# zqs01/ASR_chinese_e2e

Hardware: AMD Instinct MI355X
Metric: training throughput (utterances/s; frames/s = x T), AISHELL-1-shaped 80-mel T=500 (higher is better)
Workload: dtype bf16; 1 GPU; configs[2]: joint CTC/attention (lambda=0.3) encoder-decoder, bf16, per-GPU batch 32, T=500, F=80, V=4232, 6 layers, d_model 512, 8x64 heads, ff 1024, dropout 0.0, fwd+loss+CER+bwd+clip+Noam/Adam per step, eager launches; global_batch=32, seq_len=500, parallelism=dp1

## Files before the change

### asr_chinese_e2e_amd/csrc/asr_common.h

```cpp
#pragma once
#include <hip/hip_runtime.h>
#include <stdint.h>
#include <stdio.h>
#include <string.h>

#include <hip/hip_ext.h>

#include "../../include/asr_hip.h"

typedef __bf16 bf16_t;
typedef __attribute__((ext_vector_type(2))) float f32x2;
typedef __attribute__((ext_vector_type(4))) float f32x4;
typedef __attribute__((ext_vector_type(16))) float f32x16;
typedef __attribute__((ext_vector_type(4))) __bf16 bf16x4;
typedef __attribute__((ext_vector_type(8))) __bf16 bf16x8;
typedef __attribute__((ext_vector_type(4))) unsigned int u32x4;
typedef __attribute__((ext_vector_type(2))) unsigned int u32x2;

#define WAVE 64

void asr_set_error(const char* fmt, ...);
int asr_deterministic(void);
enum { ASR_OPT_CU_LIMIT = 0, ASR_OPT_TN_MULTI = 1, ASR_OPT_SDPA_PAIR = 2, ASR_OPT_SDPA_SMALL = 3, ASR_OPT_COUNT = 4 };
int asr_option(int key);
int asr_option_set(int key, int value);
#define ASR_FAIL(code, ...)        \
    do {                           \
        asr_set_error(__VA_ARGS__); \
        return (code);             \
    } while (0)
#define ASR_CHECK_LAUNCH(name)                                                        \
    do {                                                                              \
        hipError_t e__ = hipGetLastError();                                           \
        if (e__ != hipSuccess) ASR_FAIL(ASR_EHIP, "%s: %s", name, hipGetErrorString(e__)); \
    } while (0)

template <typename T> __device__ __forceinline__ float to_f32(T v);
template <> __device__ __forceinline__ float to_f32<float>(float v) { return v; }
template <> __device__ __forceinline__ float to_f32<bf16_t>(bf16_t v) { return (float)v; }
template <typename T> __device__ __forceinline__ T from_f32(float v);
template <> __device__ __forceinline__ float from_f32<float>(float v) { return v; }
template <> __device__ __forceinline__ bf16_t from_f32<bf16_t>(float v) { return (bf16_t)v; }

template <typename T> __device__ __forceinline__ f32x4 load4(const T* p);
template <> __device__ __forceinline__ f32x4 load4<float>(const float* p) { return *(const f32x4*)p; }
template <> __device__ __forceinline__ f32x4 load4<bf16_t>(const bf16_t* p) {
    bf16x4 v = *(const bf16x4*)p;
    f32x4 r = {(float)v[0], (float)v[1], (float)v[2], (float)v[3]};
    return r;
}
template <typename V> __device__ __forceinline__ void stream_store(V v, V* p) { __builtin_nontemporal_store(v, p); }
template <typename T> __device__ __forceinline__ void store4(T* p, f32x4 v);
template <> __device__ __forceinline__ void store4<float>(float* p, f32x4 v) { *(f32x4*)p = v; }
template <> __device__ __forceinline__ void store4<bf16_t>(bf16_t* p, f32x4 v) {
    bf16x4 r = {(bf16_t)v[0], (bf16_t)v[1], (bf16_t)v[2], (bf16_t)v[3]};
    *(bf16x4*)p = r;
}
template <typename T> __device__ __forceinline__ void load8(const T* p, float (&r)[8]);
template <> __device__ __forceinline__ void load8<float>(const float* p, float (&r)[8]) {
    f32x4 a = *(const f32x4*)p, b = *(const f32x4*)(p + 4);
#pragma unroll
    for (int i = 0; i < 4; ++i) { r[i] = a[i]; r[4 + i] = b[i]; }
}
template <> __device__ __forceinline__ void load8<bf16_t>(const bf16_t* p, float (&r)[8]) {
    bf16x8 v = *(const bf16x8*)p;
#pragma unroll
    for (int i = 0; i < 8; ++i) r[i] = (float)v[i];
}
template <typename T> __device__ __forceinline__ void store8(T* p, const float (&r)[8]);
template <> __device__ __forceinline__ void store8<float>(float* p, const float (&r)[8]) {
    f32x4 a = {r[0], r[1], r[2], r[3]}, b = {r[4], r[5], r[6], r[7]};
    *(f32x4*)p = a;
    *(f32x4*)(p + 4) = b;
}
template <> __device__ __forceinline__ void store8<bf16_t>(bf16_t* p, const float (&r)[8]) {
    bf16x8 v;
#pragma unroll
    for (int i = 0; i < 8; ++i) v[i] = (bf16_t)r[i];
    *(bf16x8*)p = v;
}

#define ASR_FULL_WAVES(threads) static_assert((threads) % 64 == 0, "wave_sum / wave_max need full 64-lane waves: block sizes must be multiples of 64")
template <int CTRL, int ROW_MASK = 0xf>
__device__ __forceinline__ float wave_dpp(float v) {
    return __int_as_float(__builtin_amdgcn_update_dpp(0, __float_as_int(v), CTRL, ROW_MASK, 0xf, true));
}
__device__ __forceinline__ float wave_sum(float v) {
    v += wave_dpp<0xB1>(v);
    v += wave_dpp<0x4E>(v);
    v += wave_dpp<0x141>(v);
    v += wave_dpp<0x140>(v);
    v += wave_dpp<0x142, 0xA>(v);
    v += wave_dpp<0x143, 0xC>(v);
    return __int_as_float(__builtin_amdgcn_readlane(__float_as_int(v), 63));
}
__device__ __forceinline__ float wave_max(float v) {
    v = fmaxf(v, __int_as_float(__builtin_amdgcn_update_dpp(__float_as_int(v), __float_as_int(v), 0xB1, 0xf, 0xf, false)));
    v = fmaxf(v, __int_as_float(__builtin_amdgcn_update_dpp(__float_as_int(v), __float_as_int(v), 0x4E, 0xf, 0xf, false)));
    v = fmaxf(v, __int_as_float(__builtin_amdgcn_update_dpp(__float_as_int(v), __float_as_int(v), 0x141, 0xf, 0xf, false)));
    v = fmaxf(v, __int_as_float(__builtin_amdgcn_update_dpp(__float_as_int(v), __float_as_int(v), 0x140, 0xf, 0xf, false)));
    v = fmaxf(v, __int_as_float(__builtin_amdgcn_update_dpp(__float_as_int(v), __float_as_int(v), 0x142, 0xA, 0xf, false)));
    v = fmaxf(v, __int_as_float(__builtin_amdgcn_update_dpp(__float_as_int(v), __float_as_int(v), 0x143, 0xC, 0xf, false)));
    return __int_as_float(__builtin_amdgcn_readlane(__float_as_int(v), 63));
}
__device__ __forceinline__ float block_sum(float v, float* red) {
    v = wave_sum(v);
// ... 91 lines not shown
```

### asr_chinese_e2e_amd/csrc/gemm.hip

```cpp
#include <stdlib.h>

#include <type_traits>

#include "asr_common.h"

namespace {

static int unsafe_debug_env(const char* name) {
#ifdef ASR_DEBUG_SWITCHES
    const char* e = getenv(name);
    return e ? atoi(e) : 0;
#else
    (void)name;
    return 0;
#endif
}

typedef __attribute__((address_space(3))) bf16x4 lds_bf16x4;
constexpr int BM = 128, BN = 128, BK = 64;
constexpr int AS = 72;

__device__ __forceinline__ int acc_row(int reg, int lane) { return (reg & 3) + 8 * (reg >> 2) + 4 * (lane >> 5); }

struct Stage4 { u32x4 v[4]; };
// ... 323 lines not shown
                            const uint32_t hi_ = ((h & 0x7fff0000u) != 0u && !(h & 0x80000000u)) ? 0xffff0000u : 0u;
                            v[q][e] &= lo_ | hi_;
                        }
                }
#pragma unroll
                for (int q = 0; q < 4; ++q) {
                    const int row = q * 8 + srow, ch = lane & 7;
                    const int m = m0 + mi * 32 + row, n = n0 + ch * 8;
                    bf16_t* rowp = C + (size_t)(m0 + mi * 32 + q * 8) * ldc + n0;
                    if constexpr (decltype(full_c)::value) stream_store(v[q], (u32x4*)((char*)rowp + lane_off));
                    else if (m < M && n + 8 <= N) stream_store(v[q], (u32x4*)((char*)rowp + lane_off));
                }
                __builtin_amdgcn_wave_barrier();
            }
        };
        if (full) store_tail(std::true_type{});
        else store_tail(std::false_type{});
    }
}

template <int ACT, bool KRAG = false>
static void launch_nt_spec(const bf16_t* a, const bf16_t* w, const float* bias, bf16_t* c, int M, int N, int K, int lda, int ldb, int ldc, hipStream_t st,
                           const bf16_t* mask = nullptr, const void* zero_page = nullptr) {
    static bool attr = false;
    if (!attr) {
        (void)hipFuncSetAttribute((const void*)gemm_nt_spec_kernel<ACT, KRAG>, hipFuncAttributeMaxDynamicSharedMemorySize, PLDS);
        attr = true;
    }
    const int t_n = ceil_div(N, PBN), t_m = ceil_div(M, PBM), ntiles = t_n * t_m;
    const int grid = ntiles < cu_count() ? ntiles : cu_count();
    asr_launch_armed(gemm_nt_spec_kernel<ACT, KRAG>, dim3(grid), dim3(512), PLDS, st, a, w, bias, c, M, N, K, lda, ldb, ldc, t_n, ntiles, mask, zero_page);
}

constexpr int SM = 64, SS = 72;
constexpr int SK = 256;
constexpr int SAS = SK + 8;
constexpr int S_A = SM * SAS;
constexpr int S_BT = SK * SS;
struct StageK { u32x4 v[8]; };
__device__ __forceinline__ void sk_load_rows(StageK& st, const bf16_t* __restrict__ base, size_t ld, int row0, int rows, int c0, int cols, int tid) {
#pragma unroll
    for (int c = 0; c < 8; ++c) {
        const int id = tid + 256 * c, row = id >> 5, ch = id & 31;
        const int gr = row0 + row, gc = c0 + ch * 8;
        const u32x4 z = {0u, 0u, 0u, 0u};
        st.v[c] = (gr < rows && gc < cols) ? *(const u32x4*)(base + (size_t)gr * ld + gc) : z;
    }
}
__device__ __forceinline__ void sk_store_rows(const StageK& st, bf16_t* tile, int tid) {
#pragma unroll
    for (int c = 0; c < 8; ++c) {
        const int id = tid + 256 * c, row = id >> 5, ch = id & 31;
        *(u32x4*)(tile + row * SAS + ch * 8) = st.v[c];
    }
}
__device__ __forceinline__ void sk_load_cols(StageK& st, const bf16_t* __restrict__ base, size_t ld, int row0, int rows, int c0, int cols, int tid) {
#pragma unroll
    for (int c = 0; c < 8; ++c) {
        const int id = tid + 256 * c, row = id >> 3, ch = id & 7;
        const int gr = row0 + row, gc = c0 + ch * 8;
        const u32x4 z = {0u, 0u, 0u, 0u};
        st.v[c] = (gr < rows && gc < cols) ? *(const u32x4*)(base + (size_t)gr * ld + gc) : z;
    }
}
__device__ __forceinline__ void sk_store_cols(const StageK& st, bf16_t* tile, int tid) {
#pragma unroll
    for (int c = 0; c < 8; ++c) {
        const int id = tid + 256 * c, row = id >> 3, ch = id & 7;
        *(u32x4*)(tile + row * SS + ch * 8) = st.v[c];
    }
}
__device__ __forceinline__ bf16x8 sm_frag_tr(const bf16_t* tile, int col0, int s, int lane) {
    const int G = lane >> 4, i = lane & 15;
    const bf16_t* p = tile + (16 * s + 8 * (G >> 1) + (i >> 2)) * SS + col0 + 16 * (G & 1) + 4 * (i & 3);
    const bf16x4 lo = __builtin_amdgcn_ds_read_tr16_b64_v4bf16((lds_bf16x4*)p);
    const bf16x4 hi = __builtin_amdgcn_ds_read_tr16_b64_v4bf16((lds_bf16x4*)(p + 4 * SS));
    return __builtin_shufflevector(lo, hi, 0, 1, 2, 3, 4, 5, 6, 7);
}

template <bool TB>
constexpr int small_lds_bytes() { return 2 * (S_A + (TB ? S_BT : S_A)) * 2; }

template <bool TB, int ACT>
__global__ __launch_bounds__(256) void gemm_small_kernel(const bf16_t* __restrict__ A, const bf16_t* __restrict__ Bm, const float* __restrict__ bias,
                                                         const bf16_t* __restrict__ mask, bf16_t* __restrict__ C, int M, int N, int K, int lda, int ldb,
                                                         int ldc, int tiles_n) {
    extern __shared__ __attribute__((aligned(16))) char smem_s[];
    constexpr int BUF = S_A + (TB ? S_BT : S_A);
    bf16_t* smem = (bf16_t*)smem_s;
    const int tid = threadIdx.x, lane = tid & 63, w = tid >> 6;
    const int tn = blockIdx.x % tiles_n, tm = blockIdx.x / tiles_n;
    const int m0 = tm * SM, n0 = tn * SM;
    const int wm = w >> 1, wn = w & 1, r = lane & 31, hh = lane >> 5;
    f32x16 acc[2];
#pragma unroll
    for (int i = 0; i < 16; ++i) { acc[0][i] = 0.f; acc[1][i] = 0.f; }
    StageK sa0, sb0, sa1, sb1;
#define SK_LOAD(SA_, SB_, K0_)                                                                 \
    {                                                                                          \
        sk_load_rows(SA_, A, lda, m0, M, (K0_), K, tid);                                       \
        if (TB) sk_load_cols(SB_, Bm, ldb, (K0_), K, n0, N, tid);    \
        else sk_load_rows(SB_, Bm, ldb, n0, N, (K0_), K, tid);       \
    }
#define SK_STORE(SA_, SB_, BUF_)                                                               \
    {                                                                                          \
        sk_store_rows(SA_, (BUF_), tid);                                                       \
        if (TB) sk_store_cols(SB_, (BUF_) + S_A, tid);                                         \
        else sk_store_rows(SB_, (BUF_) + S_A, tid);                                            \
    }
#define SK_MMA(KT_)                                                                                                                   \
    {                                                                                                                                 \
        const bf16_t* As = smem + ((KT_) & 1) * BUF;                                                                                  \
        const bf16_t* Bs = As + S_A;                                                                                                  \
             \
             \
        _Pragma("unroll") for (int ks = 0; ks < SK / 16; ++ks) {                                                                      \
            const bf16x8 af = *(const bf16x8*)(As + (wm * 32 + r) * SAS + 16 * ks + 8 * hh);                                          \
            const bf16x8 bf = TB ? sm_frag_tr(Bs, wn * 32, ks, lane) : *(const bf16x8*)(Bs + (wn * 32 + r) * SAS + 16 * ks + 8 * hh); \
            acc[ks & 1] = __builtin_amdgcn_mfma_f32_32x32x16_bf16(bf, af, acc[ks & 1], 0, 0, 0);                                      \
        }                                                                                                                             \
    }
    const int nk = (K + SK - 1) / SK;
    SK_LOAD(sa0, sb0, 0);
    if (nk > 1) SK_LOAD(sa1, sb1, SK);
    SK_STORE(sa0, sb0, smem);
    __syncthreads();
    for (int kt = 0; kt < nk; kt += 2) {
        if (kt + 2 < nk) SK_LOAD(sa0, sb0, (kt + 2) * SK);
        SK_MMA(kt);
        if (kt + 1 < nk) SK_STORE(sa1, sb1, smem + BUF);
        __syncthreads();
        if (kt + 1 >= nk) break;
        if (kt + 3 < nk) SK_LOAD(sa1, sb1, (kt + 3) * SK);
        SK_MMA(kt + 1);
        if (kt + 2 < nk) SK_STORE(sa0, sb0, smem);
        __syncthreads();
    }
#undef SK_LOAD
#undef SK_STORE
#undef SK_MMA
    const int m = m0 + wm * 32 + r;
    if (m >= M) return;
#pragma unroll
    for (int g4 = 0; g4 < 4; ++g4) {
        const int n = n0 + wn * 32 + 8 * g4 + 4 * hh;
        if (n >= N) continue;
        f32x4 o;
#pragma unroll
        for (int e = 0; e < 4; ++e) {
            float x = acc[0][4 * g4 + e] + acc[1][4 * g4 + e] + (bias ? bias[n + e] : 0.f);
            if (ACT == ASR_ACT_RELU) x = fmaxf(x, 0.f);
            o[e] = x;
        }
        if (ACT == ASR_ACT_RELU_MASK) {
            const f32x4 h4 = load4<bf16_t>(mask + (size_t)m * ldc + n);
#pragma unroll
            for (int e = 0; e < 4; ++e) o[e] = h4[e] > 0.f ? o[e] : 0.f;
        }
        store4<bf16_t>(C + (size_t)m * ldc + n, o);
    }
}

constexpr int TM = 64;

constexpr int TSTAGE = 2 * TM * 256;
__device__ __attribute__((aligned(256))) unsigned tn_zero_page[64];

template <int OFF>
__device__ __forceinline__ bf16x4 lds_tr16(unsigned addr) {
    bf16x4 v;
    asm volatile("ds_read_b64_tr_b16 %0, %1 offset:%2" : "=v"(v) : "v"(addr), "n"(OFF) : "memory");
    return v;
}
__device__ __forceinline__ unsigned tn_frag_off(int col0, int lane) {
    const int G = lane >> 4, i = lane & 15;
    const int row = 4 * (G >> 1) + (i >> 2);
    const int chunk = ((col0 >> 3) + 2 * (G & 1) + ((i & 3) >> 1)) ^ (4 * ((i >> 2) & 3));
    return (unsigned)(row * 256 + (chunk << 4) + 8 * (i & 1));
}
template <int S>
__device__ __forceinline__ bf16x8 tn_frag_swz(unsigned addr) {
    const bf16x4 lo = lds_tr16<S * 4096>(addr), hi = lds_tr16<S * 4096 + 2048>(addr);
    return __builtin_shufflevector(lo, hi, 0, 1, 2, 3, 4, 5, 6, 7);
}

template <int TRING>
__device__ __forceinline__ void tn_dma_tile(char* smem_t, const bf16_t* __restrict__ dY, const bf16_t* __restrict__ X, float* __restrict__ dW, int N, int K, int ldy,
                                            int ldx, int ldw, int n0, int k0, int tk, int mbeg, int mend, int use_atomic, const void* __restrict__ zero_page,
                                            float* __restrict__ dbias, int split, int bias_split_stride) {
    const int tid = threadIdx.x, lane = tid & 63, w = __builtin_amdgcn_readfirstlane(tid >> 6);
    constexpr int SR = TM;
    constexpr int SBYTES = TSTAGE;
    const int nsteps = (mend - mbeg + SR - 1) / SR;
    if (nsteps <= 0) return;
    const int wn = w >> 1, wk = w & 1;

    const int lrow = lane >> 4, slot = lane & 15;
    const bool is_y = w < 2;
    const bf16_t* cur[8];
    int prow[8];
#pragma unroll
    for (int j = 0; j < 8; ++j) {
        const int gg = (w & 1) * 8 + j;
        const int row = 4 * gg + lrow;
        const int col = (slot ^ (4 * (row & 3))) * 8;
        prow[j] = row;
        cur[j] = is_y ? dY + (size_t)(mbeg + row) * ldy + min(n0 + col, N - 8) : X + (size_t)(mbeg + row) * ldx + min(k0 + col, K - 8);
    }
    const size_t stage_step = (size_t)SR * (is_y ? ldy : ldx);
    const bool ragged = ((mend - mbeg) % SR) != 0;
    int it = 0, it_slot = 0;
    auto fix_last = [&]() {
        if (ragged && it == nsteps - 1) {
#pragma unroll
            for (int j = 0; j < 8; ++j) cur[j] = (mbeg + it * SR + prow[j] < mend) ? cur[j] : (const bf16_t*)zero_page;
        }
    };
    fix_last();
    auto dma = [&](int j) {
        __builtin_amdgcn_global_load_lds((gbl_void_t*)cur[j], (lds_void_t*)(smem_t + it_slot * SBYTES + (w * 8 + j) * 1024), 16, 0, 0);
    };
    auto advance = [&]() {
        ++it;
        it_slot = it_slot == TRING - 1 ? 0 : it_slot + 1;
#pragma unroll
        for (int j = 0; j < 8; ++j) cur[j] += stage_step;
        fix_last();
    };

    f32x16 acc[2][2];
#pragma unroll
    for (int a = 0; a < 2; ++a)
#pragma unroll
        for (int b = 0; b < 2; ++b)
#pragma unroll
            for (int e = 0; e < 16; ++e) acc[a][b][e] = 0.f;
    const unsigned lds_base = (unsigned)(size_t)(__attribute__((address_space(3))) char*)smem_t;
    const unsigned y_off[2] = {tn_frag_off(wn * 64, lane), tn_frag_off(wn * 64 + 32, lane)};
// ... 410 lines not shown
#pragma unroll
            for (int e = 0; e < 4; ++e) t[e] += v[e];
        }
        const size_t n = (i * 4) / K, k = i * 4 - n * K;
        float* dst = dW + n * ldw + k;
#pragma unroll
        for (int e = 0; e < 4; ++e) dst[e] = accumulate ? dst[e] + t[e] : t[e];
    }
}

static int tn_splits(int M, int N, int K) {
    const int tiles = ceil_div(N, 128) * ceil_div(K, 128);
    int s = ceil_div(256, tiles);
    const int max_s = ceil_div(M, 4 * TM);
    if (s > max_s) s = max_s;
    if (s < 1) s = 1;
    return s;
}

}

extern "C" int asr_gemm_nt_bf16(const void* A, const void* W, const float* bias, const void* res, void* C, int M, int N, int K, int lda, int ldb, int ldc,
                                int act, void* stream) {
    if (!A || !W || !C) ASR_FAIL(ASR_EINVAL, "asr_gemm_nt_bf16: null pointer");
    if (M <= 0 || N <= 0 || K <= 0) ASR_FAIL(ASR_EINVAL, "asr_gemm_nt_bf16: bad shape M=%d N=%d K=%d", M, N, K);
    if (K % 8 || lda % 8 || ldb % 8 || ldc % 4 || lda < K || ldb < K || ldc < N) ASR_FAIL(ASR_EINVAL, "asr_gemm_nt_bf16: K, lda, ldb must be multiples of 8 and ldc of 4 (K=%d lda=%d ldb=%d ldc=%d)", K, lda, ldb, ldc);
    if ((((uintptr_t)A | (uintptr_t)W) % 16) || ((uintptr_t)C % 8) || (res && (uintptr_t)res % 8) || (bias && (uintptr_t)bias % 16)) ASR_FAIL(ASR_EINVAL, "asr_gemm_nt_bf16: misaligned pointer");
    hipStream_t st = (hipStream_t)stream;
    if (act != ASR_ACT_RELU && act != ASR_ACT_NONE && act != ASR_ACT_RELU_MASK) ASR_FAIL(ASR_EINVAL, "asr_gemm_nt_bf16: unknown activation %d", act);
    const bool rows16 = N % 8 == 0 && ldc % 8 == 0 && ((uintptr_t)C % 16) == 0;
    if (act == ASR_ACT_RELU_MASK) {
        if (!res || (uintptr_t)res % 16 || K % DBK || K < 2 * PBK || !rows16)
            ASR_FAIL(ASR_EINVAL, "asr_gemm_nt_bf16: ASR_ACT_RELU_MASK needs the mask in `res`, K %% 64 == 0, K >= 128, N, ldc %% 8 == 0 and 16-byte aligned pointers");
        if (bias) ASR_FAIL(ASR_EINVAL, "asr_gemm_nt_bf16: ASR_ACT_RELU_MASK takes no bias");
        launch_nt_spec<ASR_ACT_RELU_MASK>((const bf16_t*)A, (const bf16_t*)W, nullptr, (bf16_t*)C, M, N, K, lda, ldb, ldc, st, (const bf16_t*)res);
        ASR_CHECK_LAUNCH("asr_gemm_nt_bf16");
        return ASR_OK;
    }
    if (res && act == ASR_ACT_NONE && !bias && K % DBK == 0 && K >= 2 * PBK && rows16 && ((uintptr_t)res % 16) == 0) {
        launch_nt_spec<NT_ACT_ADD_RES>((const bf16_t*)A, (const bf16_t*)W, nullptr, (bf16_t*)C, M, N, K, lda, ldb, ldc, st, (const bf16_t*)res);
        ASR_CHECK_LAUNCH("asr_gemm_nt_bf16");
        return ASR_OK;
    }
    if (K % DBK != 0 && K > PBK && !res && act == ASR_ACT_NONE && rows16) {
        static void* zero_page = nullptr;
        if (!zero_page && (hipGetSymbolAddress(&zero_page, HIP_SYMBOL(tn_zero_page)) != hipSuccess || !zero_page))
            ASR_FAIL(ASR_EINVAL, "asr_gemm_nt_bf16: zero page symbol not found");
        launch_nt_spec<ASR_ACT_NONE, true>((const bf16_t*)A, (const bf16_t*)W, bias, (bf16_t*)C, M, N, K, lda, ldb, ldc, st, nullptr, zero_page);
        ASR_CHECK_LAUNCH("asr_gemm_nt_bf16");
        return ASR_OK;
    }
    if (K % DBK == 0 && K >= 2 * PBK && !res && rows16) {
        if (act == ASR_ACT_RELU) launch_nt_spec<ASR_ACT_RELU>((const bf16_t*)A, (const bf16_t*)W, bias, (bf16_t*)C, M, N, K, lda, ldb, ldc, st);
        else launch_nt_spec<ASR_ACT_NONE>((const bf16_t*)A, (const bf16_t*)W, bias, (bf16_t*)C, M, N, K, lda, ldb, ldc, st);
        ASR_CHECK_LAUNCH("asr_gemm_nt_bf16");
        return ASR_OK;
    }
    const int tiles_n = ceil_div(N, BN), tiles_m = ceil_div(M, BM);
    if (act == ASR_ACT_RELU)
        gemm_nt_kernel<ASR_ACT_RELU><<<tiles_n * tiles_m, 256, 0, st>>>((const bf16_t*)A, (const bf16_t*)W, bias, (const bf16_t*)res, (bf16_t*)C, M, N, K, lda, ldb, ldc, tiles_n);
    else if (act == ASR_ACT_NONE)
        gemm_nt_kernel<ASR_ACT_NONE><<<tiles_n * tiles_m, 256, 0, st>>>((const bf16_t*)A, (const bf16_t*)W, bias, (const bf16_t*)res, (bf16_t*)C, M, N, K, lda, ldb, ldc, tiles_n);
    else
        ASR_FAIL(ASR_EINVAL, "asr_gemm_nt_bf16: unknown activation %d", act);
    ASR_CHECK_LAUNCH("asr_gemm_nt_bf16");
    return ASR_OK;
}

extern "C" int asr_gemm_small_bf16(const void* A, const void* Bm, const float* bias, const void* mask, void* C, int M, int N, int K, int lda, int ldb, int ldc,
                                   int trans_b, int act, void* stream) {
    if (!A || !Bm || !C) ASR_FAIL(ASR_EINVAL, "asr_gemm_small_bf16: null pointer");
    if (M <= 0 || N <= 0 || K <= 0) ASR_FAIL(ASR_EINVAL, "asr_gemm_small_bf16: bad shape M=%d N=%d K=%d", M, N, K);
    if (N % 8 || K % 8 || lda % 8 || ldb % 8 || ldc % 4 || lda < K || ldc < N || ldb < (trans_b ? N : K))
        ASR_FAIL(ASR_EINVAL, "asr_gemm_small_bf16: N, K, lda, ldb must be multiples of 8, ldc of 4 (N=%d K=%d lda=%d ldb=%d ldc=%d)", N, K, lda, ldb, ldc);
    if ((((uintptr_t)A | (uintptr_t)Bm) % 16) || ((uintptr_t)C % 8) || (mask && (uintptr_t)mask % 8) || (bias && (uintptr_t)bias % 4)) ASR_FAIL(ASR_EINVAL, "asr_gemm_small_bf16: misaligned pointer");
    if (act != ASR_ACT_NONE && act != ASR_ACT_RELU && act != ASR_ACT_RELU_MASK) ASR_FAIL(ASR_EINVAL, "asr_gemm_small_bf16: unknown activation %d", act);
    if ((act == ASR_ACT_RELU_MASK) != (mask != nullptr)) ASR_FAIL(ASR_EINVAL, "asr_gemm_small_bf16: ASR_ACT_RELU_MASK needs the activations in `mask` (and only it)");
    hipStream_t st = (hipStream_t)stream;
    const int tiles_n = ceil_div(N, SM), grid = tiles_n * ceil_div(M, SM);
    const bf16_t *a = (const bf16_t*)A, *b = (const bf16_t*)Bm, *mk = (const bf16_t*)mask;
    bf16_t* c = (bf16_t*)C;
    static bool attr = false;
    if (!attr) {
        (void)hipFuncSetAttribute((const void*)gemm_small_kernel<true, ASR_ACT_RELU_MASK>, hipFuncAttributeMaxDynamicSharedMemorySize, small_lds_bytes<true>());
        (void)hipFuncSetAttribute((const void*)gemm_small_kernel<true, ASR_ACT_RELU>, hipFuncAttributeMaxDynamicSharedMemorySize, small_lds_bytes<true>());
        (void)hipFuncSetAttribute((const void*)gemm_small_kernel<true, ASR_ACT_NONE>, hipFuncAttributeMaxDynamicSharedMemorySize, small_lds_bytes<true>());
        (void)hipFuncSetAttribute((const void*)gemm_small_kernel<false, ASR_ACT_RELU_MASK>, hipFuncAttributeMaxDynamicSharedMemorySize, small_lds_bytes<false>());
        (void)hipFuncSetAttribute((const void*)gemm_small_kernel<false, ASR_ACT_RELU>, hipFuncAttributeMaxDynamicSharedMemorySize, small_lds_bytes<false>());
        (void)hipFuncSetAttribute((const void*)gemm_small_kernel<false, ASR_ACT_NONE>, hipFuncAttributeMaxDynamicSharedMemorySize, small_lds_bytes<false>());
        attr = true;
    }
#define SMALL(TB_, ACT_) asr_launch_armed(gemm_small_kernel<TB_, ACT_>, dim3(grid), dim3(256), small_lds_bytes<TB_>(), st, a, b, bias, mk, c, M, N, K, lda, ldb, ldc, tiles_n)
    if (trans_b) {
        if (act == ASR_ACT_RELU_MASK) SMALL(true, ASR_ACT_RELU_MASK);
        else if (act == ASR_ACT_RELU) SMALL(true, ASR_ACT_RELU);
        else SMALL(true, ASR_ACT_NONE);
    } else {
        if (act == ASR_ACT_RELU_MASK) SMALL(false, ASR_ACT_RELU_MASK);
        else if (act == ASR_ACT_RELU) SMALL(false, ASR_ACT_RELU);
        else SMALL(false, ASR_ACT_NONE);
    }
#undef SMALL
    ASR_CHECK_LAUNCH("asr_gemm_small_bf16");
    return ASR_OK;
}

namespace {
static void tn_stagger(int M, int rows_per_split, int nsplit, int* r0, int* skew) {
    *r0 = rows_per_split;
    *skew = 0;
    if (nsplit >= 3) {
        int sk = (int)((long long)rows_per_split * 50 / 100 / (nsplit - 1)) / TM * TM;
        const int tri = nsplit * (nsplit - 1) / 2;
        int r = ceil_div(ceil_div(M - sk * tri > 0 ? M - sk * tri : M, nsplit), TM) * TM;
        if (sk <= 0 || r < 4 * TM || r * (nsplit - 1) + sk * ((nsplit - 1) * (nsplit - 2) / 2) >= M) return;
        *r0 = r;
        *skew = sk;
    }
}

static bool tn_multi_launch(const asr_tn_problem* probs, int nprob, int accumulate, hipStream_t st, void* zero_page) {
    if (!asr_option(ASR_OPT_TN_MULTI) || nprob > TNM_MAX || probs[0].M < 4096) return false;
    TnMulti g;
    memset(&g, 0, sizeof(g));
    int tiles = 0;
    for (int i = 0; i < nprob; ++i) {
        const asr_tn_problem& q = probs[i];
        if (q.M != probs[0].M) return false;
        TnMultiProb& t = g.p[i];
        t.dY = (const bf16_t*)q.dY; t.X = (const bf16_t*)q.X; t.dW = q.dW; t.dbias = q.dbias;
        t.N = q.N; t.K = q.K; t.ldy = q.ldy; t.ldx = q.ldx; t.ldw = q.ldw;
        t.tiles_k = ceil_div(q.K, 128);
        t.tiles = ceil_div(q.N, 128) * t.tiles_k;
        tiles += t.tiles;
    }
    const int cus = cu_count(), M = probs[0].M;
    int splits = cus / tiles;
    const int max_s = ceil_div(M, 4 * TM);
    if (splits > max_s) splits = max_s;
    if (splits < 1) splits = 1;
    if (tiles * splits * 5 < cus * 4 && splits < max_s) return false;
    const int rows_per_split = ceil_div(ceil_div(M, splits), TM) * TM;
    g.nsplit = ceil_div(M, rows_per_split);
    g.nprob = nprob;
    g.M = M;
    tn_stagger(M, rows_per_split, g.nsplit, &g.r0, &g.skew);
    int begin = 0;
    for (int i = 0; i < nprob; ++i) {
        g.p[i].block_begin = begin;
        begin += g.p[i].tiles * g.nsplit;
        if (!accumulate) {
            const size_t total = (size_t)g.p[i].N * g.p[i].K;
            const int zg = (int)((total + 255) / 256);
            zero_f32_kernel<<<zg < 1024 ? zg : 1024, 256, 0, st>>>(g.p[i].dW, g.p[i].N, g.p[i].K, g.p[i].ldw);
        }
    }
    static bool attr = false;
    if (!attr) { (void)hipFuncSetAttribute((const void*)gemm_tn_multi_kernel<3>, hipFuncAttributeMaxDynamicSharedMemorySize, 3 * TSTAGE); attr = true; }
    gemm_tn_multi_kernel<3><<<begin, 256, 3 * TSTAGE, st>>>(g, zero_page);
    return true;
}
}

extern "C" int asr_gemm_tn_grouped_bf16(const asr_tn_problem* probs, int nprob, int accumulate, void* stream) {
    if (!probs || nprob <= 0 || nprob > TG_MAX) ASR_FAIL(ASR_EINVAL, "asr_gemm_tn_grouped_bf16: 1..%d problems per call (got %d)", TG_MAX, nprob);
    if (asr_deterministic()) ASR_FAIL(ASR_EINVAL, "asr_gemm_tn_grouped_bf16: the grouped kernel combines splits with fp32 atomics - in deterministic mode call asr_gemm_tn_bias_bf16 per problem");
    hipStream_t st = (hipStream_t)stream;
    TnGroup g;
    memset(&g, 0, sizeof(g));
    g.nprob = nprob;
    long long work = 0;
    int max_m = 0;
    for (int i = 0; i < nprob; ++i) {
        const asr_tn_problem& q = probs[i];
        if (!q.dY || !q.X || !q.dW) ASR_FAIL(ASR_EINVAL, "asr_gemm_tn_grouped_bf16: null pointer in problem %d", i);
// ... 143 lines not shown
```

### asr_chinese_e2e_amd/csrc/misc.hip

```cpp
#include <stdarg.h>
#include <stdlib.h>

#include "asr_common.h"

static thread_local char g_err[512] = "";

void asr_set_error(const char* fmt, ...) {
    va_list ap;
    va_start(ap, fmt);
    vsnprintf(g_err, sizeof(g_err), fmt, ap);
    va_end(ap);
}

extern "C" int asr_abi_version(void) { return ASR_ABI_VERSION; }

static int g_deterministic = -1;
int asr_deterministic(void) {
    if (g_deterministic < 0) {
        const char* e = getenv("ASR_DETERMINISTIC");
        g_deterministic = (e && atoi(e) != 0) ? 1 : 0;
    }
    return g_deterministic;
}
extern "C" int asr_get_deterministic(void) { return asr_deterministic(); }
extern "C" int asr_set_deterministic(int on) {
    const int old = asr_deterministic();
    g_deterministic = on ? 1 : 0;
    return old;
}

static const char* const g_opt_names[ASR_OPT_COUNT] = {"cu_limit", "tn_multi", "sdpa_pair", "sdpa_small"};
static int g_opt_val[ASR_OPT_COUNT] = {0, 1, 0, 1};
static void opt_init() {}
int asr_option(int key) {
    opt_init();
    return (key >= 0 && key < ASR_OPT_COUNT) ? g_opt_val[key] : 0;
}
int asr_option_set(int key, int value) {
    opt_init();
    if (key < 0 || key >= ASR_OPT_COUNT) return 0;
    const int old = g_opt_val[key];
    g_opt_val[key] = value;
    return old;
}
extern "C" int asr_set_option(const char* name, int value, int* previous) {
    opt_init();
    if (!name) ASR_FAIL(ASR_EINVAL, "asr_set_option: null name");
    for (int i = 0; i < ASR_OPT_COUNT; ++i)
        if (strcmp(name, g_opt_names[i]) == 0) {
            if (previous) *previous = g_opt_val[i];
            g_opt_val[i] = value;
            return ASR_OK;
        }
    ASR_FAIL(ASR_EINVAL, "asr_set_option: unknown option '%s'", name);
}

extern "C" int asr_last_error(char* buf, size_t n) {
    if (buf && n) {
        strncpy(buf, g_err, n - 1);
        buf[n - 1] = 0;
    }
    return (int)strlen(g_err);
}

static unsigned fork_event_flags() { return hipEventDisableTiming | hipEventReleaseToDevice; }
static hipEvent_t g_fork_events[256];
static unsigned g_fork_next = 0;
static bool g_fork_init = false;
extern "C" int asr_stream_fork(void* from_stream, void* to_stream) {
    if (!g_fork_init) {
        for (int i = 0; i < 256; ++i)
            if (hipEventCreateWithFlags(&g_fork_events[i], fork_event_flags()) != hipSuccess) ASR_FAIL(ASR_EHIP, "asr_stream_fork: hipEventCreateWithFlags failed");
        g_fork_init = true;
    }
    hipEvent_t ev = g_fork_events[g_fork_next++ & 255u];
    hipError_t e = hipEventRecord(ev, (hipStream_t)from_stream);
    if (e == hipSuccess) e = hipStreamWaitEvent((hipStream_t)to_stream, ev, 0);
    if (e != hipSuccess) ASR_FAIL(ASR_EHIP, "asr_stream_fork: %s", hipGetErrorString(e));
    return ASR_OK;
}

static hipStream_t g_arm_from = nullptr, g_arm_to = nullptr;
static bool g_arm_set = false;
extern "C" int asr_stream_arm(void* from_stream, void* to_stream) {
    if (!g_fork_init) {
        for (int i = 0; i < 256; ++i)
            if (hipEventCreateWithFlags(&g_fork_events[i], fork_event_flags()) != hipSuccess) ASR_FAIL(ASR_EHIP, "asr_stream_arm: hipEventCreateWithFlags failed");
        g_fork_init = true;
    }
    g_arm_from = (hipStream_t)from_stream;
    g_arm_to = (hipStream_t)to_stream;
    g_arm_set = true;
    return ASR_OK;
}
extern "C" int asr_stream_arm_pending(void) {
    const int p = g_arm_set ? 1 : 0;
    g_arm_set = false;
    return p;
}
bool asr_arm_take(hipStream_t st, hipStream_t* to, hipEvent_t* ev) {
    if (!g_arm_set || st != g_arm_from) return false;
    g_arm_set = false;
    *to = g_arm_to;
    *ev = g_fork_events[g_fork_next++ & 255u];
    return true;
}

extern "C" int asr_stream_create(int priority, void** out_stream) {
    if (!out_stream) ASR_FAIL(ASR_EINVAL, "asr_stream_create: null output");
    int least = 0, greatest = 0;
    hipError_t e = hipDeviceGetStreamPriorityRange(&least, &greatest);
    if (e != hipSuccess) ASR_FAIL(ASR_EHIP, "asr_stream_create: %s", hipGetErrorString(e));
    const int prio = priority < 0 ? least : priority > 0 ? greatest : 0;
    hipStream_t st = nullptr;
    e = hipStreamCreateWithPriority(&st, hipStreamNonBlocking, prio);
// ... 612 lines not shown
```

Measured before the change: 7045 utterances/s.

## Add 4-deep register-ring prefetch variant of small GEMM kernel, enabled by default

Adds a new small-tile GEMM kernel that keeps four stages of global loads in flight in registers, feeding a double-buffered LDS. It also interleaves MFMA with LDS fragment reads through sched_group_barrier and hoists bias and ReLU-mask loads ahead of the main loop. The aim is to hide global-memory latency for the many small GEMMs in the step. The old kernel is kept as a fallback behind a new option that defaults to on, and it is also used when offsets could overflow 32 bits. The cost is higher register pressure and a lot of per-K-count template specialisation.

Measured after the change: 7223 utterances/s, median of 6. +2.5%, better.

```diff
diff --git a/asr_chinese_e2e_amd/csrc/asr_common.h b/asr_chinese_e2e_amd/csrc/asr_common.h
--- a/asr_chinese_e2e_amd/csrc/asr_common.h
+++ b/asr_chinese_e2e_amd/csrc/asr_common.h
@@ -21,7 +21,7 @@
 
 void asr_set_error(const char* fmt, ...);
 int asr_deterministic(void);
-enum { ASR_OPT_CU_LIMIT = 0, ASR_OPT_TN_MULTI = 1, ASR_OPT_SDPA_PAIR = 2, ASR_OPT_SDPA_SMALL = 3, ASR_OPT_COUNT = 4 };
+enum { ASR_OPT_CU_LIMIT = 0, ASR_OPT_TN_MULTI = 1, ASR_OPT_SDPA_PAIR = 2, ASR_OPT_SDPA_SMALL = 3, ASR_OPT_GEMM_SMALL_RING = 4, ASR_OPT_COUNT = 5 };
 int asr_option(int key);
 int asr_option_set(int key, int value);
 #define ASR_FAIL(code, ...)        \
diff --git a/asr_chinese_e2e_amd/csrc/gemm.hip b/asr_chinese_e2e_amd/csrc/gemm.hip
--- a/asr_chinese_e2e_amd/csrc/gemm.hip
+++ b/asr_chinese_e2e_amd/csrc/gemm.hip
@@ -429,9 +429,9 @@
 constexpr int small_lds_bytes() { return 2 * (S_A + (TB ? S_BT : S_A)) * 2; }
 
 template <bool TB, int ACT>
-__global__ __launch_bounds__(256) void gemm_small_kernel(const bf16_t* __restrict__ A, const bf16_t* __restrict__ Bm, const float* __restrict__ bias,
-                                                         const bf16_t* __restrict__ mask, bf16_t* __restrict__ C, int M, int N, int K, int lda, int ldb,
-                                                         int ldc, int tiles_n) {
+__global__ __launch_bounds__(256) void gemm_small_d2_kernel(const bf16_t* __restrict__ A, const bf16_t* __restrict__ Bm, const float* __restrict__ bias,
+                                                            const bf16_t* __restrict__ mask, bf16_t* __restrict__ C, int M, int N, int K, int lda, int ldb,
+                                                            int ldc, int tiles_n) {
     extern __shared__ __attribute__((aligned(16))) char smem_s[];
     constexpr int BUF = S_A + (TB ? S_BT : S_A);
     bf16_t* smem = (bf16_t*)smem_s;
@@ -501,6 +501,200 @@
         }
         if (ACT == ASR_ACT_RELU_MASK) {
             const f32x4 h4 = load4<bf16_t>(mask + (size_t)m * ldc + n);
+#pragma unroll
+            for (int e = 0; e < 4; ++e) o[e] = h4[e] > 0.f ? o[e] : 0.f;
+        }
+        store4<bf16_t>(C + (size_t)m * ldc + n, o);
+    }
+}
+
+constexpr int SD = 4;
+template <bool TB, int PF>
+struct SmallCtx {
+    const bf16_t *A, *Bm;
+    bf16_t* smem;
+    int K, lda, ldb;
+    int a_row, a_max;
+    int b_row, b_max;
+    int b_col;
+    int ch8;
+    int st_a, st_b;
+    int fr_a, fr_b;
+};
+__device__ __forceinline__ int sr_fresh(int x) {
+    asm volatile("" : "+v"(x));
+    return x;
+}
+__device__ __forceinline__ void sr_load_rows(StageK& st, const bf16_t* __restrict__ base, int ld, int row, int row_max, int k0, int ch8, int K) {
+    const int ro = sr_fresh(row), gc = min(k0 + ch8, K - 8);
+#pragma unroll
+    for (int c = 0; c < 8; ++c) st.v[c] = *(const u32x4*)(base + (unsigned)(min(ro + 8 * c * ld, row_max) + gc));
+}
+__device__ __forceinline__ void sr_load_cols(StageK& st, const bf16_t* __restrict__ base, int ld, int row, int row_max, int k0, int col) {
+    const int ro = sr_fresh(row) + k0 * ld;
+#pragma unroll
+    for (int c = 0; c < 8; ++c) st.v[c] = *(const u32x4*)(base + (unsigned)(min(ro + 32 * c * ld, row_max) + col));
+}
+__device__ __forceinline__ void sr_store_rows(const StageK& st, bf16_t* tile, int off, int kleft, int ch8) {
+    bf16_t* t = tile + sr_fresh(off);
+#pragma unroll
+    for (int c = 0; c < 8; ++c) *(u32x4*)(t + 8 * c * SAS) = st.v[c];
+    if (kleft >= SK) return;
+    const u32x4 z = {0u, 0u, 0u, 0u};
+    if (ch8 >= kleft) {
+#pragma unroll
+        for (int c = 0; c < 8; ++c) *(u32x4*)(t + 8 * c * SAS) = z;
+    }
+}
+__device__ __forceinline__ void sr_store_cols(const StageK& st, bf16_t* tile, int off, int kleft, int row) {
+    bf16_t* t = tile + sr_fresh(off);
+#pragma unroll
+    for (int c = 0; c < 8; ++c) *(u32x4*)(t + 32 * c * SS) = st.v[c];
+    if (kleft >= SK) return;
+    const u32x4 z = {0u, 0u, 0u, 0u};
+#pragma unroll
+    for (int c = 0; c < 8; ++c)
+        if (row + 32 * c >= kleft) *(u32x4*)(t + 32 * c * SS) = z;
+}
+template <bool TB, int PF>
+__device__ __forceinline__ void sr_load(const SmallCtx<TB, PF>& c, StageK& a, StageK& b, int kt) {
+    sr_load_rows(a, c.A, c.lda, c.a_row, c.a_max, kt * SK, c.ch8, c.K);
+    if (TB) sr_load_cols(b, c.Bm, c.ldb, c.b_row, c.b_max, kt * SK, c.b_col);
+    else sr_load_rows(b, c.Bm, c.ldb, c.b_row, c.b_max, kt * SK, c.ch8, c.K);
+    __builtin_amdgcn_sched_barrier(0);
+}
+template <bool TB, int PF>
+__device__ __forceinline__ void sr_store(const SmallCtx<TB, PF>& c, const StageK& a, const StageK& b, int buf, int kt) {
+    constexpr int BUF = S_A + (TB ? S_BT : S_A);
+    bf16_t* t = c.smem + buf * BUF;
+    const int kleft = c.K - kt * SK;
+    sr_store_rows(a, t, c.st_a, kleft, c.ch8);
+    if (TB) sr_store_cols(b, t + S_A, c.st_b, kleft, threadIdx.x >> 3);
+    else sr_store_rows(b, t + S_A, c.st_b, kleft, c.ch8);
+}
+template <bool TB>
+__device__ __forceinline__ void sr_frag(const bf16_t* As, const bf16_t* Bs, int ks, bf16x8& af, bf16x8& bf) {
+    af = *(const bf16x8*)(As + 16 * ks);
+    if (TB) {
+        const bf16x4 lo = __builtin_amdgcn_ds_read_tr16_b64_v4bf16((lds_bf16x4*)(Bs + 16 * ks * SS));
+        const bf16x4 hi = __builtin_amdgcn_ds_read_tr16_b64_v4bf16((lds_bf16x4*)(Bs + (16 * ks + 4) * SS));
+        bf = __builtin_shufflevector(lo, hi, 0, 1, 2, 3, 4, 5, 6, 7);
+    } else {
+        bf = *(const bf16x8*)(Bs + 16 * ks);
+    }
+}
+template <bool TB, int SPF>
+__device__ __forceinline__ void sr_mma(const SmallCtx<TB, SPF>& c, f32x16 (&acc)[2], int buf) {
+    constexpr int BUF = S_A + (TB ? S_BT : S_A);
+    constexpr int NR = TB ? 3 : 2;
+    const bf16_t* As = c.smem + buf * BUF + sr_fresh(c.fr_a);
+    const bf16_t* Bs = c.smem + buf * BUF + S_A + sr_fresh(c.fr_b);
+    bf16x8 af[SPF], bf[SPF];
+#pragma unroll
+    for (int ks = 0; ks < SPF; ++ks) sr_frag<TB>(As, Bs, ks, af[ks], bf[ks]);
+#pragma unroll
+    for (int ks = 0; ks < SK / 16; ++ks) {
+        acc[ks & 1] = __builtin_amdgcn_mfma_f32_32x32x16_bf16(bf[ks % SPF], af[ks % SPF], acc[ks & 1], 0, 0, 0);
+        if (ks + SPF < SK / 16) sr_frag<TB>(As, Bs, ks + SPF, af[ks % SPF], bf[ks % SPF]);
+    }
+    __builtin_amdgcn_sched_group_barrier(0x100, NR * SPF, 0);
+#pragma unroll
+    for (int ks = 0; ks < SK / 16; ++ks) {
+        __builtin_amdgcn_sched_group_barrier(0x008, 1, 0);
+        if (ks + SPF < SK / 16) __builtin_amdgcn_sched_group_barrier(0x100, NR, 0);
+    }
+    __builtin_amdgcn_sched_barrier(0);
+}
+template <bool TB, int R, bool FIRST, int PF>
+__device__ __forceinline__ void sr_run(const SmallCtx<TB, PF>& c, StageK (&sa)[SD], StageK (&sb)[SD], f32x16 (&acc)[2], int kt) {
+    if (FIRST) {
+#pragma unroll
+        for (int j = 0; j < (R < SD ? R : SD); ++j) sr_load<TB>(c, sa[j], sb[j], j);
+        sr_store<TB>(c, sa[0], sb[0], 0, 0);
+        __syncthreads();
+    }
+#pragma unroll
+    for (int j = 0; j < R; ++j) {
+        if (j + SD < R) sr_load<TB>(c, sa[j % SD], sb[j % SD], kt + j + SD);
+        sr_mma<TB>(c, acc, j & 1);
+        if (j + 1 < R) sr_store<TB>(c, sa[(j + 1) % SD], sb[(j + 1) % SD], (j + 1) & 1, kt + j + 1);
+        __syncthreads();
+    }
+}
+
+template <bool TB, int ACT>
+__global__ __launch_bounds__(256) void gemm_small_kernel(const bf16_t* __restrict__ A, const bf16_t* __restrict__ Bm, const float* __restrict__ bias,
+                                                         const bf16_t* __restrict__ mask, bf16_t* __restrict__ C, int M, int N, int K, int lda, int ldb,
+                                                         int ldc, int tiles_n) {
+    extern __shared__ __attribute__((aligned(16))) char smem_s[];
+    const int tid = threadIdx.x, lane = tid & 63, w = __builtin_amdgcn_readfirstlane(tid >> 6);
+    const int tn = blockIdx.x % tiles_n, tm = blockIdx.x / tiles_n;
+    const int m0 = tm * SM, n0 = tn * SM;
+    const int wm = w >> 1, wn = w & 1, r = lane & 31, hh = lane >> 5;
+    const int G = lane >> 4, i16 = lane & 15;
+    const SmallCtx<TB, ACT == ASR_ACT_RELU_MASK ? 3 : 4> c = {A, Bm, (bf16_t*)smem_s, K, lda, ldb,
+                            (m0 + (tid >> 5)) * lda, (M - 1) * lda,
+                            TB ? (tid >> 3) * ldb : (n0 + (tid >> 5)) * ldb, TB ? (K - 1) * ldb : (N - 1) * ldb,
+                            min(n0 + (tid & 7) * 8, N - 8), (tid & 31) * 8,
+                            (tid >> 5) * SAS + (tid & 31) * 8, TB ? (tid >> 3) * SS + (tid & 7) * 8 : (tid >> 5) * SAS + (tid & 31) * 8,
+                            (wm * 32 + r) * SAS + 8 * hh,
+                            TB ? (8 * (G >> 1) + (i16 >> 2)) * SS + wn * 32 + 16 * (G & 1) + 4 * (i16 & 3) : (wn * 32 + r) * SAS + 8 * hh};
+    const int m = m0 + wm * 32 + r, nb = n0 + wn * 32 + 4 * hh;
+    f32x8u bs[4];
+    u32x2 hm[4];
+#pragma unroll
+    for (int g4 = 0; g4 < 4; ++g4) {
+        const f32x8u z8 = {0.f, 0.f, 0.f, 0.f, 0.f, 0.f, 0.f, 0.f};
+        bs[g4] = bias ? *(const f32x8u*)(bias + min(n0 + wn * 32 + 8 * g4, N - 8)) : z8;
+    }
+    if (ACT == ASR_ACT_RELU_MASK) {
+#pragma unroll
+        for (int g4 = 0; g4 < 4; ++g4) hm[g4] = *(const u32x2*)(mask + (size_t)min(m, M - 1) * ldc + min(nb + 8 * g4, N - 4));
+    }
+    f32x16 acc[2];
+#pragma unroll
+    for (int i = 0; i < 16; ++i) { acc[0][i] = 0.f; acc[1][i] = 0.f; }
+    StageK sa[SD], sb[SD];
+    const int nk = (K + SK - 1) / SK;
+    if (nk == 1) sr_run<TB, 1, true>(c, sa, sb, acc, 0);
+    else if (nk == 2) sr_run<TB, 2, true>(c, sa, sb, acc, 0);
+    else if (nk == 3) sr_run<TB, 3, true>(c, sa, sb, acc, 0);
+    else {
+#pragma unroll
+        for (int j = 0; j < SD; ++j) sr_load<TB>(c, sa[j], sb[j], j);
+        sr_store<TB>(c, sa[0], sb[0], 0, 0);
+        __syncthreads();
+        int kt = 0;
+        for (; kt + 2 * SD <= nk; kt += SD) {
+#pragma unroll
+            for (int j = 0; j < SD; ++j) {
+                sr_load<TB>(c, sa[j], sb[j], kt + j + SD);
+                sr_mma<TB>(c, acc, j & 1);
+                sr_store<TB>(c, sa[(j + 1) % SD], sb[(j + 1) % SD], (j + 1) & 1, kt + j + 1);
+                __syncthreads();
+            }
+        }
+        const int left = nk - kt;
+        if (left == 4) sr_run<TB, 4, false>(c, sa, sb, acc, kt);
+        else if (left == 5) sr_run<TB, 5, false>(c, sa, sb, acc, kt);
+        else if (left == 6) sr_run<TB, 6, false>(c, sa, sb, acc, kt);
+        else sr_run<TB, 7, false>(c, sa, sb, acc, kt);
+    }
+    if (m >= M) return;
+#pragma unroll
+    for (int g4 = 0; g4 < 4; ++g4) {
+        const int n = nb + 8 * g4;
+        if (n >= N) continue;
+        f32x4 o;
+#pragma unroll
+        for (int e = 0; e < 4; ++e) {
+            float x = acc[0][4 * g4 + e] + acc[1][4 * g4 + e] + (hh ? bs[g4][4 + e] : bs[g4][e]);
+            if (ACT == ASR_ACT_RELU) x = fmaxf(x, 0.f);
+            o[e] = x;
+        }
+        if (ACT == ASR_ACT_RELU_MASK) {
+            const float h4[4] = {__uint_as_float(hm[g4][0] << 16), __uint_as_float(hm[g4][0] & 0xffff0000u), __uint_as_float(hm[g4][1] << 16),
+                                 __uint_as_float(hm[g4][1] & 0xffff0000u)};
 #pragma unroll
             for (int e = 0; e < 4; ++e) o[e] = h4[e] > 0.f ? o[e] : 0.f;
         }
@@ -1077,15 +1271,23 @@
     bf16_t* c = (bf16_t*)C;
     static bool attr = false;
     if (!attr) {
-        (void)hipFuncSetAttribute((const void*)gemm_small_kernel<true, ASR_ACT_RELU_MASK>, hipFuncAttributeMaxDynamicSharedMemorySize, small_lds_bytes<true>());
-        (void)hipFuncSetAttribute((const void*)gemm_small_kernel<true, ASR_ACT_RELU>, hipFuncAttributeMaxDynamicSharedMemorySize, small_lds_bytes<true>());
-        (void)hipFuncSetAttribute((const void*)gemm_small_kernel<true, ASR_ACT_NONE>, hipFuncAttributeMaxDynamicSharedMemorySize, small_lds_bytes<true>());
-        (void)hipFuncSetAttribute((const void*)gemm_small_kernel<false, ASR_ACT_RELU_MASK>, hipFuncAttributeMaxDynamicSharedMemorySize, small_lds_bytes<false>());
-        (void)hipFuncSetAttribute((const void*)gemm_small_kernel<false, ASR_ACT_RELU>, hipFuncAttributeMaxDynamicSharedMemorySize, small_lds_bytes<false>());
-        (void)hipFuncSetAttribute((const void*)gemm_small_kernel<false, ASR_ACT_NONE>, hipFuncAttributeMaxDynamicSharedMemorySize, small_lds_bytes<false>());
+#define SMALL_ATTR(TB_, ACT_)                                                                                                                       \
+    (void)hipFuncSetAttribute((const void*)gemm_small_kernel<TB_, ACT_>, hipFuncAttributeMaxDynamicSharedMemorySize, small_lds_bytes<TB_>());      \
+    (void)hipFuncSetAttribute((const void*)gemm_small_d2_kernel<TB_, ACT_>, hipFuncAttributeMaxDynamicSharedMemorySize, small_lds_bytes<TB_>())
+        SMALL_ATTR(true, ASR_ACT_RELU_MASK);
+        SMALL_ATTR(true, ASR_ACT_RELU);
+        SMALL_ATTR(true, ASR_ACT_NONE);
+        SMALL_ATTR(false, ASR_ACT_RELU_MASK);
+        SMALL_ATTR(false, ASR_ACT_RELU);
+        SMALL_ATTR(false, ASR_ACT_NONE);
+#undef SMALL_ATTR
         attr = true;
     }
-#define SMALL(TB_, ACT_) asr_launch_armed(gemm_small_kernel<TB_, ACT_>, dim3(grid), dim3(256), small_lds_bytes<TB_>(), st, a, b, bias, mk, c, M, N, K, lda, ldb, ldc, tiles_n)
+    const long long lim = 1ll << 31;
+    const bool ring = asr_option(ASR_OPT_GEMM_SMALL_RING) != 0 && ((long long)M + SM) * lda < lim && ((long long)(trans_b ? K : N) + SK) * ldb < lim;
+#define SMALL(TB_, ACT_)                                                                                                                                       \
+    asr_launch_armed(ring ? gemm_small_kernel<TB_, ACT_> : gemm_small_d2_kernel<TB_, ACT_>, dim3(grid), dim3(256), small_lds_bytes<TB_>(), st, a, b, bias, mk, \
+                     c, M, N, K, lda, ldb, ldc, tiles_n)
     if (trans_b) {
         if (act == ASR_ACT_RELU_MASK) SMALL(true, ASR_ACT_RELU_MASK);
         else if (act == ASR_ACT_RELU) SMALL(true, ASR_ACT_RELU);
diff --git a/asr_chinese_e2e_amd/csrc/misc.hip b/asr_chinese_e2e_amd/csrc/misc.hip
--- a/asr_chinese_e2e_amd/csrc/misc.hip
+++ b/asr_chinese_e2e_amd/csrc/misc.hip
@@ -29,8 +29,8 @@
     return old;
 }
 
-static const char* const g_opt_names[ASR_OPT_COUNT] = {"cu_limit", "tn_multi", "sdpa_pair", "sdpa_small"};
-static int g_opt_val[ASR_OPT_COUNT] = {0, 1, 0, 1};
+static const char* const g_opt_names[ASR_OPT_COUNT] = {"cu_limit", "tn_multi", "sdpa_pair", "sdpa_small", "gemm_small_ring"};
+static int g_opt_val[ASR_OPT_COUNT] = {0, 1, 0, 1, 1};
 static void opt_init() {}
 int asr_option(int key) {
     opt_init();
```
